# Multi-resolution-diffusion-recommender/SDRM

Measured on AMD Instinct MI355X. Metric: denoising-steps/sec (train+sample) on ML-1M latents, higher is better.
Workload: dtype f32; 1 GPU; ML-1M/MLP shaped synthetic latents (C3/C4); latent=340, width=340, hidden_layers=1, global_batch=8192, n_sample=5429, step_mix=15 train : 78 sample per job cycle, rng=philox4x32-10 on device, sampler_row_chains=2, parallelism=user-sharded dp1, collectives=none

## Files before the change

sdrm_amd/csrc/gemm.h:

```cpp
#pragma once
#include <hip/hip_runtime.h>
#include <stdint.h>

#include "bufres.h"

#include <type_traits>

#include "philox.h"
#include "select.h"

namespace sdrm {

typedef float f32x16 __attribute__((ext_vector_type(16)));

enum : int { LD_KCONTIG = 0, LD_MCONTIG = 1 };
enum : int { XF_NONE = 0, XF_PRELU = 1 };
enum : int {
  EPI_BIAS = 0,
  EPI_BIAS_TANH = 1,
  EPI_BIAS_TANH_G = 2,
  EPI_DPRELU = 3,
  EPI_SLAB = 4,
  EPI_PLAIN = 5,
  EPI_TANH_REV = 6,
  EPI_BIAS_G = 7,
  EPI_BIAS_ROWTAB = 9,
  EPI_BIAS_PRELU = 10
};

constexpr int NTHREADS = 256;

#ifndef SDRM_DIAG
#define SDRM_DIAG 0
#endif
#define DIAG_LD(x) do { if (!(SDRM_DIAG & 1)) { x; } } while (0)
#define DIAG_ST(x) do { if (!(SDRM_DIAG & 2)) { x; } } while (0)
#define DIAG_BAR() do { if (!(SDRM_DIAG & 4)) __syncthreads(); } while (0)

template <int BM_, int BN_, int WM_, int WN_, int MINW_ = 4, int BK_ = 16, int MF_ = 32, int PF_ = 2>
struct TileCfg {
  static constexpr int BM = BM_, BN = BN_, WM = WM_, WN = WN_, BK = BK_, MF = MF_, PF = PF_;
  static constexpr int MINW = MINW_;
  static constexpr int TM = BM_ / WM_ / MF_, TN = BN_ / WN_ / MF_;
  static constexpr int PADMAX = (MF_ == 32) ? 4 : 16;
  static constexpr int LDA = BM_ + PADMAX, LDB = BN_ + PADMAX;
  static constexpr int LDK = BK_ + 4;
  static constexpr int STAGE_KMAJOR = BK * (LDA + LDB), STAGE_KMINOR = (BM_ + BN_) * LDK;
  static constexpr int STAGE = STAGE_KMAJOR > STAGE_KMINOR ? STAGE_KMAJOR : STAGE_KMINOR;
  static_assert(WM_ * WN_ == 4, "4 waves per work-group");
  static_assert(MF_ == 32 || MF_ == 16, "MFMA tile edge");
  static_assert(TM >= 1 && TN >= 1, "wave tile must hold at least one MFMA tile");
};

template <int MF> struct AccT;
template <> struct AccT<32> { typedef float type __attribute__((ext_vector_type(16))); };
template <> struct AccT<16> { typedef float type __attribute__((ext_vector_type(4))); };

struct GemmArgs {
  const float* A; int lda; int limA;
  const float* B; int ldb; int limB;
  float* C; int ldc;
  int K;
  int kchunk;
  int tiles_n;
  int nblocks;
  int nsplits;
  uint32_t magic_tiles_n, magic_nblocks;
  const float* bias;
  const float* slopeA;
  const float* slopeB;
  const float* aux; int ldaux; const float* slopeE; float* slope_partial;
  size_t slab_stride; float* dbias; int dbias_stride;
  unsigned long long* stamps;
  int rows_valid, cols_valid;
  float* revX; float* revU; int rev_ldx, rev_s0, rev_n, rev_L, rev_step;
  float rev_c1, rev_sqrt_alpha, rev_sqrt_beta, rev_nd;
  uint32_t rev_seed_lo, rev_seed_hi, rev_call_id; int64_t rev_row0;
  const int* rev_rowid;
  const int* trow; int trow_B, ldtab;
};

__device__ __forceinline__ float prelu_f(float v, float a) { return v > 0.f ? v : a * v; }

__device__ __forceinline__ float tanh_fast(float x) {
  const float e = __builtin_amdgcn_exp2f(x * 2.885390081777927f);
  return 1.f - 2.f * __builtin_amdgcn_rcpf(e + 1.f);
}

template <int LOAD, int ROWS, int BK>
__device__ __forceinline__ void tile_offsets(int ld, uint32_t (&vo)[ROWS * BK / 4 / NTHREADS], int tid) {
  constexpr int NV = ROWS * BK / 4 / NTHREADS;
  constexpr int KQ = BK / 4;
#pragma unroll
  for (int s = 0; s < NV; ++s) {
    const int f = tid + s * NTHREADS;
    if (LOAD == LD_KCONTIG) {
      const int i = f / KQ, kq = f % KQ;
      vo[s] = (uint32_t)(i * ld + 4 * kq) * 4u;
    } else {
      constexpr int VPR = ROWS / 4;
      const int k = f / VPR, iq = f - k * VPR;
      vo[s] = (uint32_t)(k * ld + 4 * iq) * 4u;
    }
  }
}
template <int LOAD, int ROWS, int BK>
__device__ __forceinline__ brsrc tile_resource(const float* __restrict__ src, int ld, int i0, int kb) {
  return make_brsrc(LOAD == LD_KCONTIG ? src + (size_t)i0 * ld + kb : src + (size_t)kb * ld + i0, 0xffffffffu);
}
template <int LOAD, int ROWS, int BK, int AUX = 0>
__device__ __forceinline__ void load_tile(brsrc res, const uint32_t (&vo)[ROWS * BK / 4 / NTHREADS], int ld, int k0 ,
                                          float4 (&r)[ROWS * BK / 4 / NTHREADS]) {
  constexpr int NV = ROWS * BK / 4 / NTHREADS;
  const uint32_t so = (LOAD == LD_KCONTIG ? (uint32_t)k0 : (uint32_t)k0 * (uint32_t)ld) * 4u;
#pragma unroll
  for (int s = 0; s < NV; ++s) {
    const f32x4_b v = bload4a<AUX>(res, vo[s], so);
    r[s] = make_float4(v[0], v[1], v[2], v[3]);
  }
}

template <int LOAD, int XF, int ROWS, int LD, int BK>
__device__ __forceinline__ void store_tile(float* __restrict__ dst, const float4 (&r)[ROWS * BK / 4 / NTHREADS],
                                           float slope, int tid) {
  constexpr int NV = ROWS * BK / 4 / NTHREADS;
  constexpr int KQ = BK / 4;
#pragma unroll
  for (int s = 0; s < NV; ++s) {
    const int f = tid + s * NTHREADS;
    float4 v = r[s];
    if (XF == XF_PRELU) {
      v.x = prelu_f(v.x, slope); v.y = prelu_f(v.y, slope); v.z = prelu_f(v.z, slope); v.w = prelu_f(v.w, slope);
    }
    if (LOAD == LD_KCONTIG) {
      const int i = f / KQ, kq = f % KQ;
      float* d = dst + (4 * kq) * LD + i;
      d[0] = v.x; d[LD] = v.y; d[2 * LD] = v.z; d[3 * LD] = v.w;
    } else {
      constexpr int VPR = ROWS / 4;
      const int k = f / VPR, iq = f - k * VPR;
      *reinterpret_cast<float4*>(dst + k * LD + 4 * iq) = v;
    }
  }
}

template <int NV>
__device__ __forceinline__ void prelu_regs(float4 (&r)[NV], float slope) {
#pragma unroll
  for (int s = 0; s < NV; ++s) {
    r[s].x = prelu_f(r[s].x, slope); r[s].y = prelu_f(r[s].y, slope);
    r[s].z = prelu_f(r[s].z, slope); r[s].w = prelu_f(r[s].w, slope);
  }
}

template <int XF, int ROWS, int LDK, int BK>
__device__ __forceinline__ void store_tile_km(float* __restrict__ dst, const float4 (&r)[ROWS * BK / 4 / NTHREADS],
                                              float slope, int tid) {
  constexpr int NV = ROWS * BK / 4 / NTHREADS;
  constexpr int KQ = BK / 4;
#pragma unroll
  for (int s = 0; s < NV; ++s) {
    const int f = tid + s * NTHREADS;
    float4 v = r[s];
    if (XF == XF_PRELU) {
      v.x = prelu_f(v.x, slope); v.y = prelu_f(v.y, slope); v.z = prelu_f(v.z, slope); v.w = prelu_f(v.w, slope);
    }
    const int i = f / KQ, kq = f % KQ;
    *reinterpret_cast<float4*>(dst + i * LDK + 4 * kq) = v;
  }
}

__host__ __device__ __forceinline__ uint32_t gemm_magic(int d) { return d <= 1 ? 0u : (uint32_t)((1ull << 32) / (uint32_t)d) + 1u; }
__device__ __forceinline__ int div_magic(int n, uint32_t m) { return m ? (int)__umulhi((uint32_t)n, m) : n; }

__host__ inline bool gemm_set_grid(GemmArgs& a, int tiles_m, int tiles_n, int splits) {
  if (tiles_m < 1 || tiles_n < 1 || splits < 1) return false;
  const uint64_t nb = (uint64_t)tiles_m * (uint64_t)tiles_n;
  if (nb >= (1ull << 31) || nb * (uint64_t)tiles_n >= (1ull << 32) || nb * nb * (uint64_t)splits >= (1ull << 32)) return false;
  a.tiles_n = tiles_n; a.nblocks = (int)nb; a.nsplits = splits;
  a.magic_tiles_n = gemm_magic(a.tiles_n); a.magic_nblocks = gemm_magic(a.nblocks);
  return true;
}

__device__ __forceinline__ int xcd_remap(int id, int n) {
  const int q = n >> 3, r = n & 7, x = id & 7, s = id >> 3;
  return (x < r ? x * (q + 1) : r * (q + 1) + (x - r) * q) + s;
}

template <int CTRL>
__device__ __forceinline__ float quad_xor(float v) {
  const int i = __float_as_int(v);
  return __int_as_float(__builtin_amdgcn_update_dpp(i, i, CTRL, 0xF, 0xF, true));
}
template <int K>
__device__ __forceinline__ uint32_t quad_bcast(uint32_t v) {
  return (uint32_t)__builtin_amdgcn_update_dpp((int)v, (int)v, K * 0x55, 0xF, 0xF, true);
}

template <class Cfg, int LOADA, int LOADB, int XFA, int XFB, int EPI, int COHA = 0>
__device__ __forceinline__ void gemm_body(const GemmArgs& p, const int bid, const int logical_in = -1) {
  constexpr int BM = Cfg::BM, BN = Cfg::BN, BK = Cfg::BK, TM = Cfg::TM, TN = Cfg::TN, MF = Cfg::MF;
  constexpr int NR = (MF == 32) ? 16 : 4;
  constexpr int KG = (MF == 32) ? 2 : 4;
  typedef typename AccT<MF>::type acc_t;
  constexpr int LDA = BM + (MF == 16 ? 16 : (LOADA == LD_KCONTIG ? 2 : 4));
  constexpr int LDB = BN + (MF == 16 ? 16 : (LOADB == LD_KCONTIG ? 2 : 4));
  constexpr bool KM = (LOADA == LD_KCONTIG && LOADB == LD_KCONTIG);
  constexpr int LDK = Cfg::LDK;
  constexpr int BOFF = KM ? BM * LDK : BK * LDA;
  constexpr int NQ = (MF == 32) ? BK / 8 : BK / 16;
  constexpr int QSTEP = (MF == 32) ? 4 : 16;
  constexpr int NVA = BM * BK / 4 / NTHREADS, NVB = BN * BK / 4 / NTHREADS;
  static_assert(NVA >= 1 && NVB >= 1, "tile too small for 256 loader threads");
  __shared__ __attribute__((aligned(16))) float smem[2 * Cfg::STAGE];
#ifdef SDRM_STAMPS
  unsigned long long t_in = __builtin_amdgcn_s_memtime(), t_pro = 0, t_loop = 0;
  unsigned long long t_ld = 0, t_land = 0;
  const unsigned long long r_in = __builtin_amdgcn_s_memrealtime();
#endif
  asm volatile("" ::"s"(p.A), "s"(p.B), "s"(p.lda), "s"(p.ldb), "s"(p.K), "s"(p.kchunk), "s"(p.tiles_n), "s"(p.nblocks),
               "s"(p.magic_tiles_n), "s"(p.limA), "s"(p.limB));
  if constexpr (EPI == EPI_TANH_REV) asm volatile("" ::"s"(p.revX), "s"(p.revU), "s"(p.rev_ldx), "s"(p.rev_s0), "s"(p.rev_n), "s"(p.bias));
  if constexpr (EPI == EPI_BIAS_PRELU) asm volatile("" ::"s"(p.bias), "s"(p.slopeE));
  const int tid = threadIdx.x;
  const int lane = tid & 63;
  const int wave = __builtin_amdgcn_readfirstlane(tid >> 6);
  const int wm = wave / Cfg::WN, wn = wave % Cfg::WN;
  const int l31 = (MF == 32) ? (lane & 31) : (lane & 15), lhi = (MF == 32) ? (lane >> 5) : (lane >> 4);

  int logical, split;
  if (EPI == EPI_SLAB) {
    const int total = p.nblocks * p.nsplits;
    if (bid >= total) return;
    const int u = xcd_remap(bid, total);
    split = div_magic(u, p.magic_nblocks);
    logical = u - split * p.nblocks;
  } else {
    logical = logical_in >= 0 ? logical_in : xcd_remap(bid, p.nblocks);
    split = 0;
  }
  const int tile_m = div_magic(logical, p.magic_tiles_n), tile_n = logical - tile_m * p.tiles_n;
  const int m0 = tile_m * BM, n0 = tile_n * BN;
  const int kb = split * p.kchunk;
  const int ke = min(kb + p.kchunk, p.K);

  const float slopeA = (XFA == XF_PRELU) ? *p.slopeA : 0.f;
  const float slopeB = (XFB == XF_PRELU) ? *p.slopeB : 0.f;

  acc_t acc[TM][TN];
#pragma unroll
  for (int a = 0; a < TM; ++a)
#pragma unroll
    for (int b = 0; b < TN; ++b)
#pragma unroll
      for (int r = 0; r < NR; ++r) acc[a][b][r] = 0.f;

  float4 ra0[NVA], rb0[NVB], ra1[NVA], rb1[NVB];
  float dbsum = 0.f;
  const bool do_dbias = (EPI == EPI_SLAB) && (p.dbias != nullptr) && (tile_n == 0) && (tid < BM);
  const int nt = (ke - kb + BK - 1) / BK;

  const int aoff = lhi * LDA + wm * (BM / Cfg::WM) + l31;
  const int boff = lhi * LDB + wn * (BN / Cfg::WN) + l31;

  const brsrc resA = tile_resource<LOADA, BM, BK>(p.A, p.lda, m0, kb), resB = tile_resource<LOADB, BN, BK>(p.B, p.ldb, n0, kb);
  uint32_t voA[NVA], voB[NVB];
  tile_offsets<LOADA, BM, BK>(p.lda, voA, tid);
  tile_offsets<LOADB, BN, BK>(p.ldb, voB, tid);
  auto ld = [&](float4 (&xa)[NVA], float4 (&xb)[NVB], int i) {
    const int k0 = kb + min(i, nt - 1) * BK;
    load_tile<LOADA, BM, BK, COHA>(resA, voA, p.lda, k0 - kb, xa);
    load_tile<LOADB, BN, BK>(resB, voB, p.ldb, k0 - kb, xb);
  };
  auto st = [&](const float4 (&xa)[NVA], const float4 (&xb)[NVB], int stage) {
    float* An = smem + stage * Cfg::STAGE;
    if constexpr (KM) {
      store_tile_km<XFA, BM, LDK, BK>(An, xa, slopeA, tid);
      store_tile_km<XFB, BN, LDK, BK>(An + BOFF, xb, slopeB, tid);
    } else {
      store_tile<LOADA, XFA, BM, LDA, BK>(An, xa, slopeA, tid);
      store_tile<LOADB, XFB, BN, LDB, BK>(An + BOFF, xb, slopeB, tid);
    }
  };
  const bool wave_active = (m0 + wm * (BM / Cfg::WM) < p.limA) && (n0 + wn * (BN / Cfg::WN) < p.limB);
  constexpr int RQ = (EPI == EPI_TANH_REV) ? NR / 4 : 1;
  float rev_z[TM][TN][RQ][4];
  uint32_t rev_kb[TM][TN][RQ];
  auto rev_draw = [&]() {
#pragma unroll
    for (int a = 0; a < TM; ++a)
#pragma unroll
      for (int b = 0; b < TN; ++b) {
        const int col = n0 + wn * (BN / Cfg::WN) + b * MF + l31;
        const int rbase = m0 + wm * (BM / Cfg::WM) + a * MF + 4 * lhi;
        const int kq = col & 3;
        const bool k0 = kq & 1, k1 = kq & 2;
#pragma unroll
        for (int h = 0; h < RQ; ++h) {
          float n[4] = {0.f, 0.f, 0.f, 0.f};
          uint32_t bits = 0u;
#ifndef SDRM_DIAG_REV_NODRAW
          if (p.rev_step > 1) {
#else
          if (p.rev_step > 1000000) {
#endif
            const int slot = p.rev_s0 + rbase + (MF == 32 ? 8 * kq + h : kq);
            const int rkey = (p.rev_rowid != nullptr && slot < p.rev_n) ? p.rev_rowid[slot] : slot;
            const U4 w = philox4x32_10((uint32_t)(p.rev_row0 + rkey), (uint32_t)(col >> 2),
                                       PURPOSE_SAMPLE_STEP | ((uint32_t)p.rev_step << 8), p.rev_call_id, p.rev_seed_lo, p.rev_seed_hi);
            box_muller(w.x, w.y, n[0], n[1]);
            box_muller(w.z, w.w, n[2], n[3]);
            bits = (w.x & 1u) | ((w.y & 1u) << 1) | ((w.z & 1u) << 2) | ((w.w & 1u) << 3);
          }
          float g;
          g = quad_xor<0xB1>(k0 ? n[0] : n[1]); if (k0) n[0] = g; else n[1] = g;
          g = quad_xor<0xB1>(k0 ? n[2] : n[3]); if (k0) n[2] = g; else n[3] = g;
          g = quad_xor<0x4E>(k1 ? n[0] : n[2]); if (k1) n[0] = g; else n[2] = g;
          g = quad_xor<0x4E>(k1 ? n[1] : n[3]); if (k1) n[1] = g; else n[3] = g;
#pragma unroll
          for (int kk = 0; kk < 4; ++kk) rev_z[a][b][h][kk] = n[kk] * p.rev_nd;
          rev_kb[a][b][h] = ((quad_bcast<0>(bits) >> kq) & 1u) | (((quad_bcast<1>(bits) >> kq) & 1u) << 1) |
                            (((quad_bcast<2>(bits) >> kq) & 1u) << 2) | (((quad_bcast<3>(bits) >> kq) & 1u) << 3);
        }
      }
  };
  constexpr bool PF_BIAS = (EPI == EPI_TANH_REV || EPI == EPI_BIAS_PRELU) && (MF == 16);
  constexpr bool PF_STATE = (EPI == EPI_TANH_REV) && (MF == 16);
  float pf_bias[TM][TN], pf_slope = 0.f;
  float pf_x[TM][TN][PF_STATE ? NR : 1];
  auto epi_prefetch = [&]() {
    if constexpr (PF_BIAS) {
      if constexpr (EPI == EPI_BIAS_PRELU) pf_slope = *p.slopeE;
#pragma unroll
      for (int a = 0; a < TM; ++a)
#pragma unroll
        for (int b = 0; b < TN; ++b) pf_bias[a][b] = p.bias[min(n0 + wn * (BN / Cfg::WN) + b * MF + l31, p.limB - 1)];
    }
// ... 364 lines not shown
```

sdrm_amd/csrc/sdrm_hip.hip:

```cpp
#include <hip/hip_runtime.h>

#include <algorithm>
#include <cmath>
#include <cstdio>
#include <cstdlib>
#include <cstring>
#include <mutex>
#include <set>
#include <string>
#include <type_traits>
#include <utility>
#include <vector>

#include "../../include/sdrm_hip.h"
#include "../../include/sdrm_hip_debug.h"
#include "compact.h"
#include "decode.h"
#include "elementwise.h"
#include "encode.h"
#include "exchange.h"
#include "feed.h"
#include "gemm.h"
#include "input_layer.h"
#include "nll.h"
// ... 360 lines not shown
  a.B = WT; a.ldb = ldwt; a.limB = Kin;
  a.C = out; a.ldc = e->WP;
  a.K = Nout; a.kchunk = Nout;
  a.aux = aux; a.ldaux = e->WP; a.slopeE = slopeE; a.slope_partial = partial;
  return launch_gemm<LD_KCONTIG, LD_KCONTIG, XF_NONE, XF_NONE, EPI_DPRELU>(a, M, Kin, 1, st, Prof{e, PC_DGRAD, flops}, cfg);
}

template <int XB>
hipError_t gemm_wgrad(const float* dC, int lddc, int Nout, const float* Act, int ldact, int Kin, const float* slopeB,
                      int Mrows, int S, int kchunk, float* slab, float* dbias, hipStream_t st, Prof pr, int cfg) {
  GemmArgs a{};
  a.A = dC; a.lda = lddc; a.limA = Nout;
  a.B = Act; a.ldb = ldact; a.limB = Kin;
  a.C = slab; a.ldc = Kin;
  a.K = Mrows; a.kchunk = kchunk;
  a.slopeB = slopeB;
  a.slab_stride = (size_t)Nout * Kin;
  a.dbias = dbias; a.dbias_stride = Nout;
  return launch_gemm<LD_MCONTIG, LD_MCONTIG, XF_NONE, XB, EPI_SLAB>(a, Nout, Kin, S, st, pr, cfg);
}

struct WgradSpec {
  const float* dC; int lddc, Nout; const float* Act; int ldact, Kin; const float* slopeB; int S, kchunk; float* slab; float* dbias;
};

hipError_t launch_wgrad_batch(sdrm_engine* e, const WgradSpec* w, int n, int Mrows, hipStream_t st, Prof pr, bool plain_b = false) {
  GemmBatch b{};
  b.n = n;
  int grid = 0;
  for (int k = 0; k < n; ++k) {
    GemmArgs& a = b.p[k];
    a.A = w[k].dC; a.lda = w[k].lddc; a.limA = w[k].Nout;
    a.B = w[k].Act; a.ldb = w[k].ldact; a.limB = w[k].Kin;
    a.C = w[k].slab; a.ldc = w[k].Kin;
    a.K = Mrows; a.kchunk = w[k].kchunk;
    a.slopeB = w[k].slopeB;
    a.slab_stride = (size_t)w[k].Nout * w[k].Kin;
    a.dbias = w[k].dbias; a.dbias_stride = w[k].Nout;
    const int tiles_m = (w[k].Nout + Cfg0::BM - 1) / Cfg0::BM, tiles_n = (w[k].Kin + Cfg0::BN - 1) / Cfg0::BN;
    if (!gemm_set_grid(a, tiles_m, tiles_n, w[k].S)) return hipErrorInvalidValue;
    if (((uint64_t)std::max(a.kchunk, 1) + 64) * (uint64_t)std::max(a.lda, a.ldb) * 4 >= (1ull << 32)) return hipErrorInvalidValue;
    b.start[k] = grid;
#ifdef SDRM_STAMPS
    a.stamps = (g_wgrad_stamps && g_stamp_class < 0) ? g_wgrad_stamps + 8 * (size_t)grid : nullptr;
#endif
    grid += round_up(a.nblocks * w[k].S, 8);
  }
  b.start[n] = grid;
#ifdef SDRM_STAMPS
  if (grid > g_wgrad_stamps_cap) for (int k = 0; k < n; ++k) b.p[k].stamps = nullptr;
  else if (g_stamp_class < 0) g_wgrad_stamps_n = grid;
#endif
  return profiled(e, pr.cls, pr.flops, st, [&] {
    if (plain_b)
      SDRM_LAUNCH(e, (gemm_batch_kernel<Cfg0, LD_MCONTIG, LD_MCONTIG, XF_NONE, XF_NONE, EPI_SLAB>), dim3((unsigned)grid),
                         dim3(NTHREADS), 0, st, b);
    else
      SDRM_LAUNCH(e, (gemm_batch_kernel<Cfg0, LD_MCONTIG, LD_MCONTIG, XF_NONE, XF_PRELU, EPI_SLAB>), dim3((unsigned)grid),
                         dim3(NTHREADS), 0, st, b);
    return hipGetLastError();
  });
}

void pick_splits(const Tuning& tn, int Mrows, int tiles_total, int& S, int& kchunk) {
  const int BK = 32;
  int max_by_rows = Mrows / (4 * BK);
  if (max_by_rows < 1) max_by_rows = 1;
  const int tiles = tiles_total < 1 ? 1 : tiles_total;
  S = tn.wgrad_round / tiles;
  if (S < 8 || round_up((Mrows + S - 1) / S, BK) > 1024) S = tn.wgrad_blocks / tiles;
  if (S < 1) S = 1;
  if (tn.wgrad_slices > 0) S = tn.wgrad_slices;
  if (S > S_MAX) S = S_MAX;
  if (S > max_by_rows) S = max_by_rows;
  kchunk = round_up((Mrows + S - 1) / S, BK);
  S = (Mrows + kchunk - 1) / kchunk;
}

int wgrad_tiles(const Tuning& tn, int Nout, int Kin) {
  const int c = pick_cfg(tn);
  return ((Nout + kCfgBM[c] - 1) / kCfgBM[c]) * ((Kin + kCfgBN[c] - 1) / kCfgBN[c]);
}

void build_jobs(sdrm_engine* e, JobTable& tab) {
  const int L = e->L, W = e->W, T = e->T, H = e->H;
  int n = 0;
  auto add = [&](int64_t off, int rows, int cols, int flat_ld, int ncols, float* dst, int dst_ld, float* dstT = nullptr, int dstT_ld = 0) -> Job& {
    Job& j = tab.j[n++];
    j.flat_off = off; j.rows = rows; j.cols = cols; j.flat_ld = flat_ld; j.ncols = ncols;
    j.dst = dst; j.dst_ld = dst_ld; j.dstT = dstT; j.dstT_ld = dstT_ld; j.dst2 = nullptr; j.dst2_ld = 0;
    j.dstF = nullptr; j.dstFT = nullptr; j.fnct = e->WP / 16; j.fklast = -1; j.fklastT = -1;
    return j;
  };
  add(e->off_we, T, T, T, e->WeP ? T : 0, e->WeP, e->TPe);
  add(e->off_be, 1, T, T, 0, nullptr, 0);
  {
    Job& j = add(e->off_w0, W, L + T, L + T, L, e->W0c, e->K0);
    j.dstF = e->W0f; j.fklast = rc_light_klast(L, e->LP);
    j.dst2 = e->W0eP; j.dst2_ld = e->TPe;
  }
  add(e->off_b0, 1, W, W, W, e->b0c, 0);
  add(e->off_a0, 1, 1, 1, 1, nullptr, 0);
  if (H >= 1) {
    Job& j = add(e->off_wh, W, W, W, W, e->Whc, e->WP, e->WhcT, e->WP);
    j.dstF = e->Whf; j.dstFT = e->WhfT; j.fklast = j.fklastT = rc_light_klast(W, e->WP);
    add(e->off_bh, 1, W, W, W, e->bhc, 0);
    add(e->off_ah, 1, 1, 1, 1, nullptr, 0);
  }
  {
    Job& j = add(e->off_wo, L, W, W, W, e->Woc, e->WP, e->WocT, e->LP);
    j.dstF = e->Wof; j.dstFT = e->WofT; j.fklast = rc_light_klast(W, e->WP); j.fklastT = rc_light_klast(L, e->LP);
  }
  add(e->off_bo, 1, L, L, L, e->boc, 0);
  tab.n = n;
}

void adam_scalars(const sdrm_engine* e, float lr, float& step_size, float& bc2_sqrt) {
  const double k = (double)e->adam_t;
  const double bc1 = 1.0 - std::pow(0.9, k), bc2 = 1.0 - std::pow(0.999, k);
  step_size = (float)((double)lr / bc1);
  bc2_sqrt = (float)std::sqrt(bc2);
}

int launch_adam(sdrm_engine* e, const float* grad, float lr, int update, hipStream_t st) {
  JobTable tab;
  build_jobs(e, tab);
  AdamArgs a{};
  a.p = e->p; a.m = e->m; a.v = e->v; a.g = grad ? grad : e->g;
  a.b1 = 0.9f; a.b2 = 0.999f; a.eps = 1e-8f; a.wd = 1e-4f; a.update = update;
  if (update) adam_scalars(e, lr, a.step_size, a.bc2_sqrt);
  int64_t biggest = 0;
  for (int k = 0; k < tab.n; ++k) biggest = std::max<int64_t>(biggest, (int64_t)tab.j[k].rows * tab.j[k].cols);
  const int gx = (int)std::min<int64_t>(1024, std::max<int64_t>(1, (biggest + 511) / 512));
  dim3 grid(gx, tab.n);
  SDRM_LAUNCH(e, k_adam, grid, dim3(256), 0, st, tab, a);
  HIP_TRY(e, hipGetLastError());
  e->tables_fresh = false;
  e->fwd_params_live = false;
  return SDRM_OK;
}

int launch_wgrad_strips(sdrm_engine* e, double flops, hipStream_t st) {
  const int H = e->H;
  Wg2Args a{};
  int ktiles[WG2_MAX_PROBLEMS], n = 0;
  auto problem = [&](const float* A, int lda, const float* B, int ldb, float* slab, int kin, size_t slab_rows) {
    a.p[n].A = A; a.p[n].lda = lda; a.p[n].B = B; a.p[n].ldb = ldb; a.p[n].slab = slab; a.p[n].ldc = kin;
    a.p[n].slab_stride = slab_rows * (size_t)kin;
    ktiles[n++] = kin / 32;
  };
  auto actk = [&](int k) { return e->act + (size_t)k * e->MPmax * e->WP; };
  problem(dpre_buf(e, 0), e->WP, e->U, e->K0, e->slab0, e->K0, (size_t)e->WP);
  problem(e->dY, e->LP, actk(H), e->WP, e->slabO, e->WP, (size_t)e->LP);
  const int units = [&] { int t = e->K0 / 32 + (H + 1) * (e->WP / 32); return (t + 3) / 4; }();
  int S = 256 / units;
  if (S < 1) S = 1;
  if (S > S_MAX) S = S_MAX;
  const int MP = e->plan.rows;
  const int kchunk = round_up((MP + S - 1) / S, WG2_BK);
  const int slices = (MP + kchunk - 1) / kchunk;
  for (int k = H; k >= 1; --k)
    problem(dpre_buf(e, k), e->WP, actk(k - 1), e->WP, e->slabH + (size_t)(k - 1) * slices * e->WP * e->WP, e->WP, (size_t)e->WP);
  if (wg2_plan(ktiles, n, a) != units) return fail(e, SDRM_ERR_SHAPE, "strip-owned weight gradients: plan does not fit");
  a.slices = slices; a.rows = MP; a.kchunk = kchunk;
  e->bwd_S0 = e->bwd_SH = e->bwd_SO = slices;
  e->bwd_strips = true;
  return with_col_tiles(e, [&](auto nt) {
    return hip_rc(e, "k_wgrad_strips", profiled(e, PC_WGRAD_STRIPS, flops, st, [&] {
      SDRM_LAUNCH(e, (k_wgrad_strips<VAL(nt)>), dim3((unsigned)(a.units * a.slices)), dim3(NTHREADS), 0, st, a);
      return hipGetLastError();
    }));
  });
}

EmbTabArgs emb_args(sdrm_engine* e) {
  EmbTabArgs a{};
  a.temb = e->temb; a.We = e->p + e->off_we; a.be = e->p + e->off_be; a.W0 = e->p + e->off_w0; a.b0 = e->p + e->off_b0;
  a.W0c = e->W0c; a.B0tab = e->B0tab;
  a.L = e->L; a.W = e->W; a.T = e->T; a.LP = e->LP; a.WP = e->WP; a.K0 = e->K0;
  a.ones_col = e->ones_col;
  return a;
}

int emb_tables(sdrm_engine* e, hipStream_t st, const float* warm = nullptr, size_t warm_floats = 0) {
  EmbTabArgs a = emb_args(e);
  a.warm = warm; a.warm_lines = warm ? (unsigned)std::min<size_t>(warm_floats / 32, 1u << 24) : 0u;
  SDRM_LAUNCH(e, k_emb_tables, dim3(e->T + 1), dim3(1024), 2 * e->T * sizeof(float), st, a);
  HIP_TRY(e, hipGetLastError());
  e->tables_fresh = true;
  return SDRM_OK;
}
int ensure_tables(sdrm_engine* e, hipStream_t st) { return e->tables_fresh ? SDRM_OK : emb_tables(e, st); }

bool skinny_net(const sdrm_engine* e) { return e->tune.skinny && e->LP <= 64 && e->WP <= 64; }
template <class F>
int with_skinny_form(sdrm_engine* e, F&& f) {
  const auto tiles = std::make_integer_sequence<int, 4>{};
  int rc = SDRM_OK;
  with_int_in<1>(std::min((e->L + 15) / 16, 4), tiles, rc, [&](auto nl) {
    return with_int_in<1>(std::min((e->W + 15) / 16, 4), tiles, rc, [&](auto nw) { return f(nl, nw); }), rc;
  });
  return rc;
}


template <class F>
int with_row_form(sdrm_engine* e, F&& f) {
  return with_col_tiles(e, [&](auto ct) { return with_bool(rc_light_klast(e->W, e->WP) >= 0, [&](auto light) { return f(ct, light); }); });
}

DgradRowsArgs dgrad_rows_args(const sdrm_engine* e, const float* G, const float* WfT, const float* pre, const float* slope, float* out,
                              float* partial) {
  DgradRowsArgs a{};
  a.G = G; a.ldg = e->WP; a.WfT = WfT; a.pre = pre; a.ldp = e->WP; a.slope = slope; a.out = out; a.ldo = e->WP; a.slope_part = partial;
  a.act = e->act ? e->act + (pre - e->pre) : nullptr; a.from_act = (e->plan.skip_pre() && a.act) ? 1 : 0;
  return a;
}

int launch_dgrad_rows(sdrm_engine* e, const float* G, const float* WfT, const float* pre, const float* slope, float* out, float* partial,
                      int groups, double flops, hipStream_t st) {
  const DgradRowsArgs a = dgrad_rows_args(e, G, WfT, pre, slope, out, partial);
  return with_row_form(e, [&](auto ct, auto light) {
    return hip_rc(e, "k_dgrad_rows", profiled(e, PC_DGRAD_ROWS, flops, st, [&] {
      SDRM_LAUNCH(e, (k_dgrad_rows<VAL(ct), VAL(light)>), dim3((unsigned)groups), dim3(NTHREADS), 0, st, a);
      return hipGetLastError();
    }));
  });
}

void dgrad_chain_args(sdrm_engine* e, const SeedArgs& seed, DgradChainArgs& ca) {
  const int H = e->H;
  ca.seed = seed; ca.nlayers = H + 1;
  ca.layer[0] = dgrad_rows_args(e, e->dY, e->WofT, pre_buf(e, H), slope_ptr(e, H), dpre_buf(e, H), e->alpha_part + (size_t)H * e->alpha_part_stride);
  for (int k = H; k >= 1; --k)
    ca.layer[H + 1 - k] = dgrad_rows_args(e, dpre_buf(e, k), e->WhfT, pre_buf(e, k - 1), slope_ptr(e, k - 1), dpre_buf(e, k - 1),
                                          e->alpha_part + (size_t)(k - 1) * e->alpha_part_stride);
}

int launch_dgrad_chain(sdrm_engine* e, const DgradChainArgs& a, int groups, double flops, hipStream_t st) {
  return with_row_form(e, [&](auto ct, auto light) {
    return hip_rc(e, "k_dgrad_chain", profiled(e, PC_DGRAD_ROWS, flops, st, [&] {
      SDRM_LAUNCH(e, (k_dgrad_chain<VAL(ct), VAL(light)>), dim3((unsigned)groups), dim3(NTHREADS), 0, st, a);
      return hipGetLastError();
    }));
  });
}

bool use_rowchain(const sdrm_engine* e, int B) {
  if (!e->W0f || e->tune.rowchain <= 0 || e->tune.force_cfg >= 0) return false;
  if (e->tune.rowchain >= 2) return true;
  const int G = (B + RC_USERS - 1) / RC_USERS;
  const int rounds = (G + 255) / 256;
  return rounds == 1 ? G >= 154 : G * 6 >= rounds * 256 * 5;
}

int chains_for(const Tuning& t, int n, int WP) {
  if (t.chains >= 1) return t.chains > 4 ? 4 : t.chains;
  return (size_t)n * (size_t)WP >= (size_t)2560 * 352 ? 2 : 1;
}

inline unsigned xabort_read(const sdrm_engine* e) { return e->xabort_host ? *(volatile const unsigned*)e->xabort_host : 0u; }
bool persist_now(const sdrm_engine* e) { return e->call.path == SampleCall::PERSIST && xabort_read(e) == 0u; }

int chains_on_aux(const sdrm_engine* e) { return e->chain_sched.detached ? 1 : e->call.chains - 1; }

int chains_join(sdrm_engine* e, hipStream_t st) {
  e->bwd_begun = false;
  if (e->chain_sched.state != ChainSched::FORKED) return SDRM_OK;
  for (int c = 0; c < chains_on_aux(e); ++c) {
    HIP_TRY(e, hipEventRecord(e->ev_join[c], e->aux[c]));
    HIP_TRY(e, hipStreamWaitEvent(st, e->ev_join[c], 0));
  }
  e->chain_sched.state = ChainSched::ON_CALLER;
  return SDRM_OK;
}

int chains_begin(sdrm_engine* e, hipStream_t st) {
  if (int jr = chains_join(e, st)) return jr;
  e->chain_sched.state = ChainSched::ON_CALLER;
  e->chain_sched.detached = false;
  return SDRM_OK;
}

int chains_train_forward(sdrm_engine* e, hipStream_t st) {
  ChainSched& s = e->chain_sched;
  const SampleCall& c = e->call;
  if (!s.train_queued) s.train_row_owned = false;
  s.train_queued = true; s.hold_marked = false;
  if (e->tune.detach > 0 && c.active && c.path != SampleCall::SKINNY && c.i_next >= 1 && c.chains == 1 && !s.detached &&
      s.state == ChainSched::ON_CALLER && !e->prof_on && !persist_now(e)) {
    HIP_TRY(e, hipEventRecord(e->ev_fork, st));
    s.state = ChainSched::DETACH_ARMED;
  }
  return SDRM_OK;
}
void chains_train_row_owned(sdrm_engine* e) { e->chain_sched.train_row_owned = true; }

int chains_wgrads_queued(sdrm_engine* e, hipStream_t st) {
  if (e->chain_sched.state != ChainSched::FORKED || !e->tune.hold_early || !e->chain_sched.train_row_owned) return SDRM_OK;
  HIP_TRY(e, hipEventRecord(e->ev_hold, st));
  e->chain_sched.hold_marked = true;
  return SDRM_OK;
}

bool chains_small_call_beside(const sdrm_engine* e) {
  return e->call.active && (e->chain_sched.state == ChainSched::DETACH_ARMED || (e->chain_sched.state == ChainSched::FORKED && e->chain_sched.detached));
}

int chains_streams(sdrm_engine* e, hipStream_t st, hipStream_t (&on)[4]) {
  ChainSched& s = e->chain_sched;
  auto aux_wait = [&](hipEvent_t ev) -> int {
    for (int c = 0; c < chains_on_aux(e); ++c) HIP_TRY(e, hipStreamWaitEvent(e->aux[c], ev, 0));
    return SDRM_OK;
  };
  auto hold = [&]() -> int {
    if (!s.train_queued || !s.train_row_owned) return SDRM_OK;
    if (s.hold_marked) { s.hold_marked = false; return aux_wait(e->ev_hold); }
    HIP_TRY(e, hipEventRecord(e->ev_fork, st));
    return aux_wait(e->ev_fork);
  };
  if (e->prof_on) {
    if (s.state == ChainSched::DETACH_ARMED) s.state = ChainSched::ON_CALLER;
// ... 2278 lines not shown
```

sdrm_amd/csrc/wgrad2.h:

```cpp
#pragma once
#include <hip/hip_runtime.h>
#include <stdint.h>

#include "bufres.h"
#include "gemm.h"

#ifndef WG2_DIAG
#define WG2_DIAG 0
#endif

namespace sdrm {

constexpr int WG2_MAX_PROBLEMS = 8;
constexpr int WG2_MAX_UNITS = 32;
constexpr int WG2_BK = 16;

struct Wg2Problem {
  const float* A; int lda;
  const float* B; int ldb;
  float* slab; int ldc;
  size_t slab_stride;
};

struct Wg2Strip { int8_t problem; int8_t ktile; };

struct Wg2Args {
  Wg2Problem p[WG2_MAX_PROBLEMS];
  Wg2Strip strip[WG2_MAX_UNITS][4];
  int units, slices, rows, kchunk;
};

__device__ __forceinline__ Wg2Problem wg2_problem(const Wg2Args& a, int idx) {
  Wg2Problem r = a.p[0];
#pragma unroll
  for (int p = 1; p < WG2_MAX_PROBLEMS; ++p)
    if (p == idx) r = a.p[p];
  return r;
}

template <int NT>
struct Wg2Cfg {
  static constexpr int WP = 32 * NT, LDA = WP + 4, LDB = 32 + 4;
  static constexpr int A_TILE = WG2_BK * LDA, B_TILE = WG2_BK * LDB;
  static constexpr int STAGE = 2 * A_TILE + 4 * B_TILE;
  static constexpr size_t LDS_BYTES = 2 * (size_t)STAGE * 4;
  static constexpr int NA4 = WG2_BK * WP / 4, NB4 = 4 * WG2_BK * 32 / 4;
  static constexpr int NLA = (NA4 + NTHREADS - 1) / NTHREADS, NLB = NB4 / NTHREADS;
  static_assert(NLB == 2, "two B blocks per half work-group");
  static_assert(LDS_BYTES <= 160 * 1024, "stages do not fit LDS");
};

template <int NT>
__global__ __launch_bounds__(NTHREADS, 1) void k_wgrad_strips(const Wg2Args a) {
  typedef Wg2Cfg<NT> C;
  constexpr int WP = C::WP, LDA = C::LDA, LDB = C::LDB, BK = WG2_BK;
  __shared__ __attribute__((aligned(16))) float smem[2 * C::STAGE];
  const int tid = threadIdx.x, lane = tid & 63;
  const int wave = __builtin_amdgcn_readfirstlane(tid >> 6);
  const int l31 = lane & 31, lhi = lane >> 5;
  const int logical = xcd_remap((int)blockIdx.x, a.units * a.slices);
  const int slice = logical / a.units, unit = logical - slice * a.units;
  const int m_begin = slice * a.kchunk, m_end = min(m_begin + a.kchunk, a.rows);
  const int nt = (m_end - m_begin) / BK;

  const Wg2Strip st = a.strip[unit][wave];
  const int pa = a.strip[unit][0].problem;
  int pb = pa;
#pragma unroll
  for (int w = 1; w < 4; ++w)
    if (a.strip[unit][w].problem >= 0) pb = a.strip[unit][w].problem;
  const bool two = pb != pa;
  const int ai = (st.problem == pa || st.problem < 0) ? 0 : 1;
  const bool active = st.problem >= 0;

  constexpr int QA = WP / 4;
  const Wg2Problem Pa = wg2_problem(a, pa), Pb = wg2_problem(a, pb);
  const int lda_a = Pa.lda, lda_b = Pb.lda;
  auto span = [&](int ld, int skip) __attribute__((always_inline)) {
    const size_t b = ((size_t)(a.rows - m_begin) * (size_t)ld - (size_t)skip) * 4;
    return (uint32_t)(b < 0xffffffffull ? b : 0xffffffffull);
  };
  const brsrc Ra = make_brsrc(Pa.A + (size_t)m_begin * lda_a, span(lda_a, 0)), Rb = make_brsrc(Pb.A + (size_t)m_begin * lda_b, span(lda_b, 0));
  brsrc RB0, RB1; int Bld[2];
  {
    const Wg2Strip s0 = a.strip[unit][(wave >> 1)], s1 = a.strip[unit][(wave >> 1) + 2];
    const Wg2Problem P0 = wg2_problem(a, s0.problem < 0 ? pa : s0.problem), P1 = wg2_problem(a, s1.problem < 0 ? pa : s1.problem);
    Bld[0] = P0.ldb; Bld[1] = P1.ldb;
    const int c0 = 32 * (s0.problem < 0 ? 0 : s0.ktile), c1 = 32 * (s1.problem < 0 ? 0 : s1.ktile);
    RB0 = make_brsrc(P0.B + (size_t)m_begin * P0.ldb + c0, span(P0.ldb, c0));
    RB1 = make_brsrc(P1.B + (size_t)m_begin * P1.ldb + c1, span(P1.ldb, c1));
  }
  struct RSet { float4 a[C::NLA], a2[C::NLA], b[C::NLB]; };
  RSet r0, r1, r2;
  auto zero = [&](RSet& r) __attribute__((always_inline)) {
#pragma unroll
    for (int j = 0; j < C::NLA; ++j) r.a[j] = r.a2[j] = make_float4(0.f, 0.f, 0.f, 0.f);
#pragma unroll
    for (int j = 0; j < C::NLB; ++j) r.b[j] = make_float4(0.f, 0.f, 0.f, 0.f);
  };
  zero(r0); zero(r1); zero(r2);
  int rowA[C::NLA], quadA[C::NLA];
#pragma unroll
  for (int j = 0; j < C::NLA; ++j) {
    const int f = min(tid + j * NTHREADS, C::NA4 - 1);
    rowA[j] = f / QA; quadA[j] = f - rowA[j] * QA;
  }
  const int rowB = (tid & 127) >> 3, quadB = tid & 7;
  uint32_t voA[C::NLA], voA2[C::NLA], voB[2];
#pragma unroll
  for (int j = 0; j < C::NLA; ++j) {
    voA[j] = (uint32_t)((rowA[j] * lda_a + 4 * quadA[j]) * 4);
    voA2[j] = (uint32_t)((rowA[j] * lda_b + 4 * quadA[j]) * 4);
  }
#pragma unroll
  for (int j = 0; j < 2; ++j) voB[j] = (uint32_t)((rowB * Bld[j] + 4 * quadB) * 4);
  auto as4 = [](f32x4_b v) __attribute__((always_inline)) { return make_float4(v[0], v[1], v[2], v[3]); };
  auto gload_piece = [&](auto two_tag, RSet& r, int m0, int k) __attribute__((always_inline)) {
    constexpr bool TWO = decltype(two_tag)::value;
    constexpr int NA = TWO ? 2 * C::NLA : C::NLA;
    if (k < C::NLA) r.a[k] = as4(bload4(Ra, voA[k], (uint32_t)((m0 - m_begin) * lda_a) * 4u));
    else if (TWO && k < NA) r.a2[k - C::NLA] = as4(bload4(Rb, voA2[k - C::NLA], (uint32_t)((m0 - m_begin) * lda_b) * 4u));
    else if (k == NA) r.b[0] = as4(bload4(RB0, voB[0], (uint32_t)((m0 - m_begin) * Bld[0]) * 4u));
    else if (k == NA + 1) r.b[1] = as4(bload4(RB1, voB[1], (uint32_t)((m0 - m_begin) * Bld[1]) * 4u));
  };
  auto lstore_piece = [&](auto two_tag, const RSet& r, float* S, int k) __attribute__((always_inline)) {
    constexpr bool TWO = decltype(two_tag)::value;
    constexpr int NA = TWO ? 2 * C::NLA : C::NLA;
    if (k < C::NLA) *reinterpret_cast<float4*>(S + rowA[k] * LDA + 4 * quadA[k]) = r.a[k];
    else if (TWO && k < NA) *reinterpret_cast<float4*>(S + C::A_TILE + rowA[k - C::NLA] * LDA + 4 * quadA[k - C::NLA]) = r.a2[k - C::NLA];
    else if (k < NA + C::NLB)
      *reinterpret_cast<float4*>(S + 2 * C::A_TILE + ((wave >> 1) + 2 * (k - NA)) * C::B_TILE + rowB * LDB + 4 * quadB) = r.b[k - NA];
  };
  auto gload = [&](auto two_tag, RSet& r, int step) __attribute__((always_inline)) {
    constexpr int NPC = (decltype(two_tag)::value ? 2 * C::NLA : C::NLA) + C::NLB;
    const int m0 = m_begin + min(step, nt - 1) * BK;
#pragma unroll
    for (int k = 0; k < NPC; ++k) gload_piece(two_tag, r, m0, k);
  };
  auto lstore = [&](auto two_tag, const RSet& r, int stage) __attribute__((always_inline)) {
    constexpr int NPC = (decltype(two_tag)::value ? 2 * C::NLA : C::NLA) + C::NLB;
#pragma unroll
    for (int k = 0; k < NPC; ++k) lstore_piece(two_tag, r, smem + stage * C::STAGE, k);
  };

  f32x16 acc[NT];
#pragma unroll
  for (int t = 0; t < NT; ++t)
#pragma unroll
    for (int r = 0; r < 16; ++r) acc[t][r] = 0.f;

  const int aoff = ai * C::A_TILE + lhi * LDA + l31;
  const int boff = 2 * C::A_TILE + wave * C::B_TILE + lhi * LDB + l31;

  auto kstep = [&](auto two_tag, int i, RSet& nx) __attribute__((always_inline)) {
    constexpr int NPC = (decltype(two_tag)::value ? 2 * C::NLA : C::NLA) + C::NLB;
    constexpr int NSLOT = (BK / 2) * NT, HALF = NSLOT / 2;
    constexpr int STRIDE = HALF / NPC >= 1 ? HALF / NPC : 1;
    static_assert(NPC <= HALF, "more staging pieces than MFMA slots");
    const float* S = smem + (i & 1) * C::STAGE;
    float* Sn = smem + ((i + 1) & 1) * C::STAGE;
    const int m4 = m_begin + min(i + 4, nt - 1) * BK;
    float fa0[NT], fa1[NT], fb0 = 0.f, fb1 = 0.f;
#pragma unroll
    for (int t = 0; t < NT; ++t) fa0[t] = S[aoff + 32 * t];
    fb0 = S[boff];
#pragma unroll
    for (int g = 0; g < BK / 2; ++g) {
      float (&ca)[NT] = (g & 1) ? fa1 : fa0;
      float (&na)[NT] = (g & 1) ? fa0 : fa1;
      const float cb = (g & 1) ? fb1 : fb0;
      float& nb = (g & 1) ? fb0 : fb1;
#pragma unroll
      for (int t = 0; t < NT; ++t) {
        if (!(WG2_DIAG & 1)) acc[t] = __builtin_amdgcn_mfma_f32_32x32x2f32(ca[t], cb, acc[t], 0, 0, 0);
        if (g + 1 < BK / 2 && !(WG2_DIAG & 8)) {
          if (t == 0) nb = S[boff + 2 * (g + 1) * LDB];
          na[t] = S[aoff + 2 * (g + 1) * LDA + 32 * t];
        }
        const int slot = g * NT + t;
        if (slot < HALF) {
          if (slot % STRIDE == 0 && slot / STRIDE < NPC && !(WG2_DIAG & 2)) lstore_piece(two_tag, nx, Sn, slot / STRIDE);
        } else {
          const int s2 = slot - HALF;
          if (s2 % STRIDE == 0 && s2 / STRIDE < NPC && !(WG2_DIAG & 4)) gload_piece(two_tag, nx, m4, s2 / STRIDE);
        }
        __builtin_amdgcn_sched_barrier(0);
      }
    }
    __syncthreads();
  };
  auto run = [&](auto two_tag) __attribute__((always_inline)) {
    gload(two_tag, r0, 0);
    lstore(two_tag, r0, 0);
    gload(two_tag, r1, 1); gload(two_tag, r2, 2); gload(two_tag, r0, 3);
    __syncthreads();
    int i = 0;
    for (; i + 2 < nt; i += 3) {
      kstep(two_tag, i, r1);
      kstep(two_tag, i + 1, r2);
      kstep(two_tag, i + 2, r0);
    }
    if (i < nt) kstep(two_tag, i, r1);
    if (i + 1 < nt) kstep(two_tag, i + 1, r2);
  };
  if (nt > 0) {
    if (two) run(std::true_type{});
    else run(std::false_type{});
  }

  if (!active) return;
  const Wg2Problem P = wg2_problem(a, st.problem);
  float* __restrict__ dst = P.slab + (size_t)slice * P.slab_stride + (size_t)(4 * lhi) * P.ldc + 32 * st.ktile + l31;
#pragma unroll
  for (int t = 0; t < NT; ++t)
#pragma unroll
    for (int r = 0; r < 16; ++r) dst[(size_t)(32 * t + (r & 3) + 8 * (r >> 2)) * P.ldc] = acc[t][r];
}

inline int wg2_plan(const int* ktiles, int nproblems, Wg2Args& a) {
  int n = 0;
  for (int p = 0; p < nproblems; ++p) n += ktiles[p];
  const int units = (n + 3) / 4;
  if (nproblems > WG2_MAX_PROBLEMS || units > WG2_MAX_UNITS) return 0;
  int u = 0, w = 0;
  for (int p = 0; p < nproblems; ++p)
    for (int k = 0; k < ktiles[p]; ++k) {
      a.strip[u][w].problem = (int8_t)p; a.strip[u][w].ktile = (int8_t)k;
      if (++w == 4) { w = 0; ++u; }
    }
  for (; w > 0 && w < 4; ++w) { a.strip[u][w].problem = -1; a.strip[u][w].ktile = 0; }
  a.units = units;
  return units;
}

}
```

Measured before the change: 9158 denoising-steps/s.

## Flatten wgrad strip scheduling into linear task list across slices

Replaces the fixed unit×slice grid for weight-gradient strips with a flat list of (problem, ktile, slice) tasks, where four consecutive tasks make one work-group. Slices now split the row steps evenly with remainders instead of rounded chunks, and the slice count can be forced through a tuning knob. The aim is to drop padded idle waves in partially filled units and balance the K-range across slices. A work-group may now straddle two slices or problems with different step counts, which costs extra buffer setup and runs the longer step count for both.

```diff
diff --git a/sdrm_amd/csrc/gemm.h b/sdrm_amd/csrc/gemm.h
--- a/sdrm_amd/csrc/gemm.h
+++ b/sdrm_amd/csrc/gemm.h
@@ -172,6 +172,7 @@
 
 __host__ __device__ __forceinline__ uint32_t gemm_magic(int d) { return d <= 1 ? 0u : (uint32_t)((1ull << 32) / (uint32_t)d) + 1u; }
 __device__ __forceinline__ int div_magic(int n, uint32_t m) { return m ? (int)__umulhi((uint32_t)n, m) : n; }
+__host__ __device__ __forceinline__ int div_magic_hd(int n, uint32_t m) { return m ? (int)(((uint64_t)(uint32_t)n * m) >> 32) : n; }
 
 __host__ inline bool gemm_set_grid(GemmArgs& a, int tiles_m, int tiles_n, int splits) {
   if (tiles_m < 1 || tiles_n < 1 || splits < 1) return false;
@@ -182,7 +183,7 @@
   return true;
 }
 
-__device__ __forceinline__ int xcd_remap(int id, int n) {
+__host__ __device__ __forceinline__ int xcd_remap(int id, int n) {
   const int q = n >> 3, r = n & 7, x = id & 7, s = id >> 3;
   return (x < r ? x * (q + 1) : r * (q + 1) + (x - r) * q) + s;
 }
diff --git a/sdrm_amd/csrc/sdrm_hip.hip b/sdrm_amd/csrc/sdrm_hip.hip
--- a/sdrm_amd/csrc/sdrm_hip.hip
+++ b/sdrm_amd/csrc/sdrm_hip.hip
@@ -536,22 +536,17 @@
   auto actk = [&](int k) { return e->act + (size_t)k * e->MPmax * e->WP; };
   problem(dpre_buf(e, 0), e->WP, e->U, e->K0, e->slab0, e->K0, (size_t)e->WP);
   problem(e->dY, e->LP, actk(H), e->WP, e->slabO, e->WP, (size_t)e->LP);
-  const int units = [&] { int t = e->K0 / 32 + (H + 1) * (e->WP / 32); return (t + 3) / 4; }();
-  int S = 256 / units;
-  if (S < 1) S = 1;
-  if (S > S_MAX) S = S_MAX;
   const int MP = e->plan.rows;
-  const int kchunk = round_up((MP + S - 1) / S, WG2_BK);
-  const int slices = (MP + kchunk - 1) / kchunk;
+  const int slices = wg2_slices(e->K0 / 32 + (H + 1) * (e->WP / 32), MP / WG2_BK, e->tune.wgrad_slices, S_MAX);
   for (int k = H; k >= 1; --k)
     problem(dpre_buf(e, k), e->WP, actk(k - 1), e->WP, e->slabH + (size_t)(k - 1) * slices * e->WP * e->WP, e->WP, (size_t)e->WP);
-  if (wg2_plan(ktiles, n, a) != units) return fail(e, SDRM_ERR_SHAPE, "strip-owned weight gradients: plan does not fit");
-  a.slices = slices; a.rows = MP; a.kchunk = kchunk;
+  const int groups = wg2_plan(ktiles, n, MP, slices, a);
+  if (groups < 1) return fail(e, SDRM_ERR_SHAPE, "strip-owned weight gradients: plan does not fit");
   e->bwd_S0 = e->bwd_SH = e->bwd_SO = slices;
   e->bwd_strips = true;
   return with_col_tiles(e, [&](auto nt) {
     return hip_rc(e, "k_wgrad_strips", profiled(e, PC_WGRAD_STRIPS, flops, st, [&] {
-      SDRM_LAUNCH(e, (k_wgrad_strips<VAL(nt)>), dim3((unsigned)(a.units * a.slices)), dim3(NTHREADS), 0, st, a);
+      SDRM_LAUNCH(e, (k_wgrad_strips<VAL(nt)>), dim3((unsigned)groups), dim3(NTHREADS), 0, st, a);
       return hipGetLastError();
     }));
   });
diff --git a/sdrm_amd/csrc/wgrad2.h b/sdrm_amd/csrc/wgrad2.h
--- a/sdrm_amd/csrc/wgrad2.h
+++ b/sdrm_amd/csrc/wgrad2.h
@@ -12,7 +12,8 @@
 namespace sdrm {
 
 constexpr int WG2_MAX_PROBLEMS = 8;
-constexpr int WG2_MAX_UNITS = 32;
+constexpr int WG2_WAVE_SLOTS = 4 * 256;
+constexpr int WG2_MIN_STRIPS = 4;
 constexpr int WG2_BK = 16;
 
 struct Wg2Problem {
@@ -22,13 +23,32 @@
   size_t slab_stride;
 };
 
-struct Wg2Strip { int8_t problem; int8_t ktile; };
+struct Wg2Task { int problem, ktile, slice; };
 
 struct Wg2Args {
   Wg2Problem p[WG2_MAX_PROBLEMS];
-  Wg2Strip strip[WG2_MAX_UNITS][4];
-  int units, slices, rows, kchunk;
+  int ktile0[WG2_MAX_PROBLEMS];
+  int P; uint32_t magic_P;
+  int slices, ksteps;
+  int q0, r0;
+  int tasks, groups;
 };
+
+__host__ __device__ __forceinline__ Wg2Task wg2_task(const Wg2Args& a, int q) {
+  Wg2Task t;
+  t.slice = div_magic_hd(q, a.magic_P);
+  const int rem = q - t.slice * a.P;
+  t.problem = 0; t.ktile = rem;
+#pragma unroll
+  for (int p = 1; p < WG2_MAX_PROBLEMS; ++p)
+    if (rem >= a.ktile0[p]) { t.problem = p; t.ktile = rem - a.ktile0[p]; }
+  if (q >= a.tasks) { t.problem = -1; t.ktile = 0; t.slice = 0; }
+  return t;
+}
+__host__ __device__ __forceinline__ int wg2_slice_begin(const Wg2Args& a, int s) { return s * a.q0 + (s < a.r0 ? s : a.r0); }
+__host__ __device__ __forceinline__ int wg2_slice_steps(const Wg2Args& a, int s) { return a.q0 + (s < a.r0 ? 1 : 0); }
+
+__host__ __device__ __forceinline__ Wg2Task wg2_last(const Wg2Args& a, int w) { return wg2_task(a, 4 * w + 3 < a.tasks ? 4 * w + 3 : a.tasks - 1); }
 
 __device__ __forceinline__ Wg2Problem wg2_problem(const Wg2Args& a, int idx) {
   Wg2Problem r = a.p[0];
@@ -58,37 +78,34 @@
   const int tid = threadIdx.x, lane = tid & 63;
   const int wave = __builtin_amdgcn_readfirstlane(tid >> 6);
   const int l31 = lane & 31, lhi = lane >> 5;
-  const int logical = xcd_remap((int)blockIdx.x, a.units * a.slices);
-  const int slice = logical / a.units, unit = logical - slice * a.units;
-  const int m_begin = slice * a.kchunk, m_end = min(m_begin + a.kchunk, a.rows);
-  const int nt = (m_end - m_begin) / BK;
-
-  const Wg2Strip st = a.strip[unit][wave];
-  const int pa = a.strip[unit][0].problem;
-  int pb = pa;
-#pragma unroll
-  for (int w = 1; w < 4; ++w)
-    if (a.strip[unit][w].problem >= 0) pb = a.strip[unit][w].problem;
-  const bool two = pb != pa;
-  const int ai = (st.problem == pa || st.problem < 0) ? 0 : 1;
+  const int logical = xcd_remap((int)blockIdx.x, a.groups);
+
+  const Wg2Task st = wg2_task(a, 4 * logical + wave), ta = wg2_task(a, 4 * logical), tb = wg2_last(a, logical);
+  const bool two = tb.problem != ta.problem || tb.slice != ta.slice;
   const bool active = st.problem >= 0;
+  const int ai = (!active || (st.problem == ta.problem && st.slice == ta.slice)) ? 0 : 1;
+  const int nt = max(wg2_slice_steps(a, ta.slice), wg2_slice_steps(a, tb.slice));
 
   constexpr int QA = WP / 4;
-  const Wg2Problem Pa = wg2_problem(a, pa), Pb = wg2_problem(a, pb);
+  const Wg2Problem Pa = wg2_problem(a, ta.problem), Pb = wg2_problem(a, tb.problem);
   const int lda_a = Pa.lda, lda_b = Pb.lda;
-  auto span = [&](int ld, int skip) __attribute__((always_inline)) {
-    const size_t b = ((size_t)(a.rows - m_begin) * (size_t)ld - (size_t)skip) * 4;
+  auto span = [&](int slice, int ld, int skip) __attribute__((always_inline)) {
+    const size_t b = ((size_t)(wg2_slice_steps(a, slice) * BK) * (size_t)ld - (size_t)skip) * 4;
     return (uint32_t)(b < 0xffffffffull ? b : 0xffffffffull);
   };
-  const brsrc Ra = make_brsrc(Pa.A + (size_t)m_begin * lda_a, span(lda_a, 0)), Rb = make_brsrc(Pb.A + (size_t)m_begin * lda_b, span(lda_b, 0));
+  auto row0 = [&](int slice) __attribute__((always_inline)) { return (size_t)(wg2_slice_begin(a, slice) * BK); };
+  const brsrc Ra = make_brsrc(Pa.A + row0(ta.slice) * lda_a, span(ta.slice, lda_a, 0));
+  const brsrc Rb = make_brsrc(Pb.A + row0(tb.slice) * lda_b, span(tb.slice, lda_b, 0));
   brsrc RB0, RB1; int Bld[2];
   {
-    const Wg2Strip s0 = a.strip[unit][(wave >> 1)], s1 = a.strip[unit][(wave >> 1) + 2];
-    const Wg2Problem P0 = wg2_problem(a, s0.problem < 0 ? pa : s0.problem), P1 = wg2_problem(a, s1.problem < 0 ? pa : s1.problem);
+    Wg2Task s0 = wg2_task(a, 4 * logical + (wave >> 1)), s1 = wg2_task(a, 4 * logical + (wave >> 1) + 2);
+    if (s0.problem < 0) { s0 = ta; s0.ktile = 0; }
+    if (s1.problem < 0) { s1 = ta; s1.ktile = 0; }
+    const Wg2Problem P0 = wg2_problem(a, s0.problem), P1 = wg2_problem(a, s1.problem);
     Bld[0] = P0.ldb; Bld[1] = P1.ldb;
-    const int c0 = 32 * (s0.problem < 0 ? 0 : s0.ktile), c1 = 32 * (s1.problem < 0 ? 0 : s1.ktile);
-    RB0 = make_brsrc(P0.B + (size_t)m_begin * P0.ldb + c0, span(P0.ldb, c0));
-    RB1 = make_brsrc(P1.B + (size_t)m_begin * P1.ldb + c1, span(P1.ldb, c1));
+    const int c0 = 32 * s0.ktile, c1 = 32 * s1.ktile;
+    RB0 = make_brsrc(P0.B + row0(s0.slice) * P0.ldb + c0, span(s0.slice, P0.ldb, c0));
+    RB1 = make_brsrc(P1.B + row0(s1.slice) * P1.ldb + c1, span(s1.slice, P1.ldb, c1));
   }
   struct RSet { float4 a[C::NLA], a2[C::NLA], b[C::NLB]; };
   RSet r0, r1, r2;
@@ -115,13 +132,13 @@
 #pragma unroll
   for (int j = 0; j < 2; ++j) voB[j] = (uint32_t)((rowB * Bld[j] + 4 * quadB) * 4);
   auto as4 = [](f32x4_b v) __attribute__((always_inline)) { return make_float4(v[0], v[1], v[2], v[3]); };
-  auto gload_piece = [&](auto two_tag, RSet& r, int m0, int k) __attribute__((always_inline)) {
+  auto gload_piece = [&](auto two_tag, RSet& r, int step, int k) __attribute__((always_inline)) {
     constexpr bool TWO = decltype(two_tag)::value;
     constexpr int NA = TWO ? 2 * C::NLA : C::NLA;
-    if (k < C::NLA) r.a[k] = as4(bload4(Ra, voA[k], (uint32_t)((m0 - m_begin) * lda_a) * 4u));
-    else if (TWO && k < NA) r.a2[k - C::NLA] = as4(bload4(Rb, voA2[k - C::NLA], (uint32_t)((m0 - m_begin) * lda_b) * 4u));
-    else if (k == NA) r.b[0] = as4(bload4(RB0, voB[0], (uint32_t)((m0 - m_begin) * Bld[0]) * 4u));
-    else if (k == NA + 1) r.b[1] = as4(bload4(RB1, voB[1], (uint32_t)((m0 - m_begin) * Bld[1]) * 4u));
+    if (k < C::NLA) r.a[k] = as4(bload4(Ra, voA[k], (uint32_t)(step * BK * lda_a) * 4u));
+    else if (TWO && k < NA) r.a2[k - C::NLA] = as4(bload4(Rb, voA2[k - C::NLA], (uint32_t)(step * BK * lda_b) * 4u));
+    else if (k == NA) r.b[0] = as4(bload4(RB0, voB[0], (uint32_t)(step * BK * Bld[0]) * 4u));
+    else if (k == NA + 1) r.b[1] = as4(bload4(RB1, voB[1], (uint32_t)(step * BK * Bld[1]) * 4u));
   };
   auto lstore_piece = [&](auto two_tag, const RSet& r, float* S, int k) __attribute__((always_inline)) {
     constexpr bool TWO = decltype(two_tag)::value;
@@ -133,9 +150,9 @@
   };
   auto gload = [&](auto two_tag, RSet& r, int step) __attribute__((always_inline)) {
     constexpr int NPC = (decltype(two_tag)::value ? 2 * C::NLA : C::NLA) + C::NLB;
-    const int m0 = m_begin + min(step, nt - 1) * BK;
-#pragma unroll
-    for (int k = 0; k < NPC; ++k) gload_piece(two_tag, r, m0, k);
+    const int i0 = min(step, nt - 1);
+#pragma unroll
+    for (int k = 0; k < NPC; ++k) gload_piece(two_tag, r, i0, k);
   };
   auto lstore = [&](auto two_tag, const RSet& r, int stage) __attribute__((always_inline)) {
     constexpr int NPC = (decltype(two_tag)::value ? 2 * C::NLA : C::NLA) + C::NLB;
@@ -159,7 +176,7 @@
     static_assert(NPC <= HALF, "more staging pieces than MFMA slots");
     const float* S = smem + (i & 1) * C::STAGE;
     float* Sn = smem + ((i + 1) & 1) * C::STAGE;
-    const int m4 = m_begin + min(i + 4, nt - 1) * BK;
+    const int i4 = min(i + 4, nt - 1);
     float fa0[NT], fa1[NT], fb0 = 0.f, fb1 = 0.f;
 #pragma unroll
     for (int t = 0; t < NT; ++t) fa0[t] = S[aoff + 32 * t];
@@ -182,7 +199,7 @@
           if (slot % STRIDE == 0 && slot / STRIDE < NPC && !(WG2_DIAG & 2)) lstore_piece(two_tag, nx, Sn, slot / STRIDE);
         } else {
           const int s2 = slot - HALF;
-          if (s2 % STRIDE == 0 && s2 / STRIDE < NPC && !(WG2_DIAG & 4)) gload_piece(two_tag, nx, m4, s2 / STRIDE);
+          if (s2 % STRIDE == 0 && s2 / STRIDE < NPC && !(WG2_DIAG & 4)) gload_piece(two_tag, nx, i4, s2 / STRIDE);
         }
         __builtin_amdgcn_sched_barrier(0);
       }
@@ -210,27 +227,33 @@
 
   if (!active) return;
   const Wg2Problem P = wg2_problem(a, st.problem);
-  float* __restrict__ dst = P.slab + (size_t)slice * P.slab_stride + (size_t)(4 * lhi) * P.ldc + 32 * st.ktile + l31;
+  float* __restrict__ dst = P.slab + (size_t)st.slice * P.slab_stride + (size_t)(4 * lhi) * P.ldc + 32 * st.ktile + l31;
 #pragma unroll
   for (int t = 0; t < NT; ++t)
 #pragma unroll
     for (int r = 0; r < 16; ++r) dst[(size_t)(32 * t + (r & 3) + 8 * (r >> 2)) * P.ldc] = acc[t][r];
 }
 
-inline int wg2_plan(const int* ktiles, int nproblems, Wg2Args& a) {
+inline int wg2_slices(int P, int ksteps, int forced, int smax) {
+  int S = forced > 0 ? forced : (WG2_WAVE_SLOTS / 4) / (P < 1 ? 1 : (P + 3) / 4);
+  if (S > smax) S = smax;
+  if (S > ksteps) S = ksteps;
+  return S < 1 ? 1 : S;
+}
+inline int wg2_plan(const int* ktiles, int nproblems, int rows, int slices, Wg2Args& a) {
+  if (nproblems < 1 || nproblems > WG2_MAX_PROBLEMS || rows < WG2_BK || rows % WG2_BK != 0) return 0;
   int n = 0;
-  for (int p = 0; p < nproblems; ++p) n += ktiles[p];
-  const int units = (n + 3) / 4;
-  if (nproblems > WG2_MAX_PROBLEMS || units > WG2_MAX_UNITS) return 0;
-  int u = 0, w = 0;
-  for (int p = 0; p < nproblems; ++p)
-    for (int k = 0; k < ktiles[p]; ++k) {
-      a.strip[u][w].problem = (int8_t)p; a.strip[u][w].ktile = (int8_t)k;
-      if (++w == 4) { w = 0; ++u; }
-    }
-  for (; w > 0 && w < 4; ++w) { a.strip[u][w].problem = -1; a.strip[u][w].ktile = 0; }
-  a.units = units;
-  return units;
-}
-
-}
+  for (int p = 0; p < nproblems; ++p) {
+    if (ktiles[p] < WG2_MIN_STRIPS) return 0;
+    a.ktile0[p] = n; n += ktiles[p];
+  }
+  for (int p = nproblems; p < WG2_MAX_PROBLEMS; ++p) a.ktile0[p] = n;
+  a.ksteps = rows / WG2_BK;
+  if (slices < 1 || slices > a.ksteps) return 0;
+  a.P = n; a.magic_P = gemm_magic(n);
+  a.slices = slices; a.q0 = a.ksteps / slices; a.r0 = a.ksteps % slices;
+  a.tasks = n * slices; a.groups = (a.tasks + 3) / 4;
+  return a.groups;
+}
+
+}
```

After: 9133 denoising-steps/s. About the same (-0.3%).
